# henrique/rsba

Measured on AMD Instinct MI355X. Metric: residual+Jacobian evals/sec, higher is better.
Workload: dtype f64; 1 GPU; C4: rolling-shutter scene, 1000 frames x 2 poses, 100000 points, 2041284 observations, HORIZONTAL shutter, calibrated; observations_total=2041284, observations_this_rank=2041284, jacobian_cols=15, partition=single GPU

## Files before the change

rsba_amd/csrc/chol_plan.cpp:

```cpp
#include "chol_plan.hpp"

#include <algorithm>

namespace rsba {

int32_t CholHostPlan::slot_of(int i, int k) const {
  if (i == k) return slot_base[k];
  auto it = std::lower_bound(col[k].begin(), col[k].end(), i);
  return (it != col[k].end() && *it == i) ? slot_base[k] + 1 + (int32_t)(it - col[k].begin()) : -1;
}

void chol_symbolic(int nt, const std::vector<std::vector<int32_t>>& adj, const TileOrder& order, CholHostPlan* hp) {
  hp->nt = nt;
  hp->perm = order.perm;
  const std::vector<int32_t>& perm = hp->perm;
  std::vector<int32_t>& iperm = hp->iperm;
  iperm.resize(nt);
  for (int k = 0; k < nt; ++k) iperm[perm[k]] = k;
  std::vector<std::vector<int32_t>>&col = hp->col, &row = hp->row;
  col.assign(nt, {}); row.assign(nt, {});
  {
    std::vector<std::vector<uint8_t>> mark(nt);
    for (int k = 0; k < nt; ++k) mark[k].assign(nt - k, 0);
    for (int t = 0; t < nt; ++t) for (int u : adj[t]) { const int i = std::max(iperm[t], iperm[u]), k = std::min(iperm[t], iperm[u]); mark[k][i - k] = 1; }
// ... 111 lines not shown
        s.sub_pub[fs] = (int32_t)(s.diag_info.size() / 4) - 1;
      } else s.diag_fuse.push_back(-1);
      sub_base[j] = (int32_t)(s.sub_info.size() / 4);
      s.back_info.push_back(slot_base[j]); s.back_info.push_back(perm[j]);
      for (auto it = col[j].rbegin(); it != col[j].rend(); ++it) { s.back_list.push_back(slot_of(*it, j)); s.back_list.push_back(perm[*it]); }
      s.back_ptr.push_back((int32_t)(s.back_list.size() / 2));
      for (int32_t i : col[j]) {
        s.sub_info.push_back(slot_of(i, j)); s.sub_info.push_back(slot_base[j]); s.sub_col.push_back(perm[j]); s.sub_pub.push_back(-1);
        if (sharded) { s.sub_info_sh.push_back(slot_of(i, j)); s.sub_info_sh.push_back(slot_base[j]); }
        sub_colnew.push_back(j);
        const int32_t sp0 = (int32_t)(s.sub_list.size() / 2);
        klev.clear(); pk.clear();
        for (int32_t k : rj) { const int32_t sik = slot_of(i, k); if (sik >= 0) { s.sub_list.push_back(sik); s.sub_list.push_back(slot_of(j, k)); klev.push_back(level[k]); if (topcol && cpart[k] >= 0) pk.push_back(cpart[k]); } }
        s.sub_ptr.push_back((int32_t)(s.sub_list.size() / 2));
        chunk_it(1, sp0, (int32_t)(s.sub_list.size() / 2), s.sub_info, s.sub_own, sp0, (int)pk.size(), pk, sharded ? &s.sub_info_sh : nullptr, slot_of(i, j));
      }
    }
    s.lev_diag_ptr.push_back((int32_t)(s.diag_info.size() / 4));
    s.lev_sub_ptr.push_back((int32_t)(s.sub_info.size() / 4));
    s.lev_upd_ptr.push_back((int32_t)(s.upd.size() / 4));
  }
  s.nparts = parts;
  auto push = [](std::vector<int32_t>& t, int kind, int item) { t.push_back(kind); t.push_back(item); };
  for (int l = 0; l < nlev; ++l) {
    for (int32_t u : upd_by_level[l]) push(s.tasks, kTaskUpdate, u);
    for (int d = s.lev_diag_ptr[l]; d < s.lev_diag_ptr[l + 1]; ++d) push(s.tasks, kTaskDiag, d);
    if (two_rhs) for (int d = s.lev_diag_ptr[l]; d < s.lev_diag_ptr[l + 1]; ++d) push(s.tasks, kTaskFwd2, d);
    for (int t = s.lev_sub_ptr[l]; t < s.lev_sub_ptr[l + 1]; ++t) push(s.tasks, kTaskSub, t);
  }
  if (two_rhs) push(s.tasks, kTaskEta, 0);
  for (int l = nlev - 1; l >= 0; --l)
    for (int d = s.lev_diag_ptr[l]; d < s.lev_diag_ptr[l + 1]; ++d) push(s.tasks, kTaskBack, d);
  s.diag_toprow.assign(diag_colnew.size(), -1);
  const int64_t T3 = (int64_t)kTile * kTile * kTile;
  s.cholesky_flops = T3 * ((int64_t)(s.diag_list.size() / 2) + 2 * (int64_t)(s.sub_list.size() / 2) + (int64_t)(s.sub_info.size() / 4)) +
                     2 * T3 / 3 * (int64_t)(s.diag_info.size() / 4) + 4 * (int64_t)kTile * kTile * ((int64_t)s.nslots + nt);
  s.row_mine.assign((size_t)nt, 1);
  if (!sharded) return;

  const int me = in.rank;
  auto mine_or_top = [&](int col_new, int kind, int item) { const int p = cpart[col_new]; if (p == me) push(s.tasks_a, kind, item); else if (p < 0) push(s.tasks_b, kind, item); };
  for (int l = 0; l < nlev; ++l) {
    for (int32_t u : upd_by_level[l]) { if (upd_owner[u] == me) push(s.tasks_a, kTaskUpdate, u); else if (upd_owner[u] < 0) push(s.tasks_b, kTaskUpdate, u); }
    for (int d = s.lev_diag_ptr[l]; d < s.lev_diag_ptr[l + 1]; ++d) mine_or_top(diag_colnew[d], kTaskDiag, d);
    if (two_rhs) for (int d = s.lev_diag_ptr[l]; d < s.lev_diag_ptr[l + 1]; ++d) mine_or_top(diag_colnew[d], kTaskFwd2, d);
    for (int t = s.lev_sub_ptr[l]; t < s.lev_sub_ptr[l + 1]; ++t) mine_or_top(sub_colnew[t], kTaskSub, t);
  }
  if (two_rhs) {
    for (int d = 0; d < (int)diag_colnew.size(); ++d) if (cpart[diag_colnew[d]] < 0) push(s.tasks_a, kTaskFwd2P, d);
    push(s.tasks_a, kTaskEta, 0);
    push(s.tasks_b, kTaskEta, 0);
  }
  for (int l = nlev - 1; l >= 0; --l)
    for (int d = s.lev_diag_ptr[l]; d < s.lev_diag_ptr[l + 1]; ++d) { const int p = cpart[diag_colnew[d]]; if (p == me || p < 0) push(s.tasks_b, kTaskBack, d); }
  {
    std::vector<int32_t> trow_of_col((size_t)nt, -1);
    int32_t cnt = 0;
    for (int j = 0; j < nt; ++j) if (cpart[j] < 0) trow_of_col[j] = cnt++;
    for (size_t d = 0; d < diag_colnew.size(); ++d) s.diag_toprow[d] = trow_of_col[diag_colnew[d]];
  }
  std::vector<uint8_t> has_pair((size_t)s.nslots, 0);
  for (size_t t = 0; t < in.pair_I->size(); ++t) { const int a = s.iperm[(*in.pair_I)[t]], b = s.iperm[(*in.pair_J)[t]]; has_pair[slot_of(std::max(a, b), std::min(a, b))] = 1; }
  s.asm_ptr.assign(1, 0);
  for (int j = 0; j < nt; ++j) if (cpart[j] < 0) {
    const int trow = (int)s.top_tiles.size();
    s.top_tiles.push_back(perm[j]);
    auto add = [&](int32_t slot, int rhs_row) {
      s.top_slots.push_back(slot); s.top_info.push_back(has_pair[slot]); s.top_info.push_back(rhs_row);
      const std::vector<int32_t>& a = asm_of_slot[slot];
      for (size_t q = 0; q + 1 < a.size(); q += 2) if (a[q] == me) s.asm_list.push_back(a[q + 1]);
// ... 16 lines not shown
```

rsba_amd/csrc/chol_plan.hpp:

```cpp
#pragma once
#include <cstdint>
#include <vector>

#include "tile_order.hpp"

namespace rsba {

enum : int { kTaskUpdate = 0, kTaskDiag = 1, kTaskSub = 2, kTaskBack = 3, kTaskFwd2 = 4, kTaskEta = 5, kTaskFwd2P = 6 };

struct CholPlanOptions {
  int chunk = 12, tail = 2;
  bool fuse_last = true;
};

struct CholTaskInput {
  const TileOrder* order = nullptr;
  bool sharded = false;
  int rank = 0;
  bool two_rhs = false;
  const std::vector<int32_t>*pair_I = nullptr, *pair_J = nullptr;
  CholPlanOptions opt;
};

struct CholHostPlan {
  int nt = 0, nslots = 0;
  std::vector<int32_t> perm, iperm;
  std::vector<std::vector<int32_t>> col, row;
  std::vector<int32_t> slot_base;
  std::vector<int32_t> slot_tiles;
  int32_t slot_of(int i, int k) const;

  bool sharded = false, two_rhs = false;
  int nlev = 0, nparts = 0;
  std::vector<int32_t> level, cpart;
  std::vector<int32_t> lev_diag_ptr, lev_sub_ptr, lev_upd_ptr;
  std::vector<int32_t> upd, upd_owner;
  std::vector<int32_t> diag_info, diag_ptr, diag_list, diag_own;
  std::vector<int32_t> diag_fuse;
  std::vector<int32_t> sub_info, sub_ptr, sub_list, sub_own;
  std::vector<int32_t> sub_col;
  std::vector<int32_t> sub_pub;
  std::vector<int32_t> back_info, back_ptr, back_list;
  std::vector<int32_t> tasks;
  std::vector<int32_t> fwd_full, diag_toprow;
  std::vector<int32_t> tasks_a, tasks_b, fwd_a, fwd_b;
  std::vector<int32_t> diag_info_sh, sub_info_sh;
  std::vector<int32_t> top_slots, top_info;
  std::vector<int32_t> asm_ptr, asm_list;
  std::vector<int32_t> top_tiles, top_fill;
  std::vector<uint8_t> row_mine, row_check, row_sep;
  int64_t cholesky_flops = 0;
  int local_levels = 0, separator_levels = 0;
};

void chol_symbolic(int nt, const std::vector<std::vector<int32_t>>& adj, const TileOrder& order, CholHostPlan* hp);
void chol_tasks(const CholTaskInput& in, CholHostPlan* hp);

}
```

rsba_amd/csrc/cholesky.hip:

```cpp
#include "solver_state.hpp"

namespace rsba {

namespace {

constexpr int T = kTile;
constexpr int TP = T + 1;

__device__ __forceinline__ double rsqrt_nr(double x) {
  double y = __builtin_amdgcn_rsq(x);
  y = y * (1.5 - 0.5 * x * y * y);
  y = y * (1.5 - 0.5 * x * y * y);
  return y;
}

__device__ __forceinline__ double* tile_ptr(const SolverDev& sv, int slot) { return sv.S + (size_t)slot * (T * T); }

__device__ __forceinline__ double readlane_f64(double v, int lane) {
  const int lo = __builtin_amdgcn_readlane(__double2loint(v), lane);
  const int hi = __builtin_amdgcn_readlane(__double2hiint(v), lane);
  return __hiloint2double(hi, lo);
}

__device__ __forceinline__ void lds_barrier() {
// ... 928 lines not shown
  switch (kind) {
    case kTaskUpdate: task_update<DAG>(sv, pl, item, smem, tid); break;
    case kTaskDiag: task_diag<DAG>(sv, pl, item, smem, tid); break;
    case kTaskSub: task_sub<DAG>(sv, pl, item, smem, tid); break;
    case kTaskFwd2: { const int tr = gl(pl.diag_toprow + item);
      task_forward<DAG>(sv, pl, item, gl(pl.fwd_range + 2 * item), gl(pl.fwd_range + 2 * item + 1), sv.border2, (pl.fwd2_minus && tr >= 0) ? pl.fwd2_minus + (size_t)tr * T : nullptr, sv.zv2, smem, tid); } break;
    case kTaskFwd2P: task_forward<DAG>(sv, pl, item, gl(pl.fwd_range + 2 * item), gl(pl.fwd_range + 2 * item + 1), sv.border2, nullptr, sv.zv2, smem, tid, pl.fwd2_partial + (size_t)gl(pl.diag_toprow + item) * T); break;
    case kTaskEta: task_eta<DAG>(sv, pl, smem, tid); break;
    default: task_back<DAG>(sv, pl, item, smem, tid); break;
  }
}

__global__ __launch_bounds__(256) void chol_level_kernel(const SolverDev sv, const CholPlan pl, int kind, int first) {
  extern __shared__ __attribute__((aligned(16))) double smem[];
  run_task<false>(sv, pl, kind, first + blockIdx.x, smem, threadIdx.x);
}

__global__ __launch_bounds__(256, 2) void chol_dag_kernel(const DagArgs* __restrict__ args) {
  extern __shared__ __attribute__((aligned(16))) double smem[];
  __shared__ int s_ticket;
  const int tid = threadIdx.x;
  const CholPlan& pl = args->pl;
  if (lm_stopped(args->sv.ctl)) return;
  for (;;) {
    lds_barrier();
    if (tid == 0) {
      const int tk = (int)__hip_atomic_fetch_add(pl.ticket, 1u, __ATOMIC_RELAXED, __HIP_MEMORY_SCOPE_AGENT);
      s_ticket = tk;
      s_trace_slot = (pl.trace && tk < pl.ntasks) ? pl.trace + 8 * (size_t)tk : nullptr;
      if (s_trace_slot) { s_trace_slot[0] = blockIdx.x; s_trace_slot[1] = s_trace_slot[2] = wall_clock64(); }
    }
    lds_barrier();
    const int t = s_ticket;
    if (t >= pl.ntasks) {
      if (tid == 0 && __hip_atomic_fetch_add(pl.ticket + 3, 1u, __ATOMIC_RELAXED, __HIP_MEMORY_SCOPE_AGENT) == gridDim.x - 1) {
        __hip_atomic_store(pl.ticket + 0, 0u, __ATOMIC_RELAXED, __HIP_MEMORY_SCOPE_AGENT);
        __hip_atomic_store(pl.ticket + 3, 0u, __ATOMIC_RELAXED, __HIP_MEMORY_SCOPE_AGENT);
      }
      return;
    }
    int task_tid = tid;
    asm volatile("" : "+v"(task_tid));
    run_task<true>(args->sv, pl, gl(pl.tasks + 2 * t), gl(pl.tasks + 2 * t + 1), smem, task_tid);
    if (tid == 0 && s_trace_slot) s_trace_slot[7] = wall_clock64();
  }
}

template <bool DAG>
__device__ __forceinline__ void task_forward(const SolverDev& sv, const CholPlan& pl, int d, int p0, int p1, const double* __restrict__ b2, const double* __restrict__ minus, double* z2,
                                             double* smem, int tid, double* partial_out) {
  constexpr int CG = 10;
  double* zb = smem;
  double* sp = smem + T;
// ... 228 lines not shown
```

rsba_amd/csrc/partition.hip:

```cpp
#include <algorithm>
#include <cstring>
#include <vector>

#include "handle.hpp"
#include "solver_state.hpp"
#include "tile_order.hpp"
#include "chol_plan.hpp"

using namespace rsba;

namespace {

int32_t partition(const rsba_problem_desc* d, int32_t world, int32_t* owner, int32_t* num_top_tiles, std::vector<int32_t>& part_of) {
  if (!d || !owner || world < 1) return rsba_set_error(RSBA_ERR_INVALID_ARGUMENT, "bad partition arguments");
  const int P = d->poses_per_frame;
  if (P != 1 && P != 2) return rsba_set_error(RSBA_ERR_INVALID_ARGUMENT, "poses_per_frame must be 1 or 2");
  const TileLayout lay(P, d->num_frames, d->calibrated != 0, d->num_intrinsics);
  const int FR = lay.FR, M = d->num_points, NIB = lay.NIB, NPF = lay.NPF, nt = lay.nt;
  const int64_t N = d->num_observations;
  if (num_top_tiles) *num_top_tiles = 0;
  if (world == 1 || N == 0) { std::fill(owner, owner + M, 0); part_of.assign(nt, 0); return RSBA_OK; }
  for (int64_t i = 0; i < N; ++i)
    if (d->obs_frame[i] < 0 || d->obs_frame[i] >= FR || d->obs_point[i] < 0 || d->obs_point[i] >= M) return rsba_set_error(RSBA_ERR_INVALID_ARGUMENT, "observation index out of range");
  auto intr_of = [&](int f) { return (NIB > 1 && d->frame_intrinsics) ? d->frame_intrinsics[f] : 0; };
// ... 69 lines not shown
}

extern "C" int32_t rsba_debug_chol_plan(int32_t nt, int32_t num_edges, const int32_t* edges, int32_t world, int32_t rank, int32_t two_rhs, int32_t chunk, int32_t tail,
                                        int32_t fuse_last, void (*emit)(void* ctx, const char* name, const int32_t* data, int64_t count), void* ctx) {
  if (nt < 1 || num_edges < 0 || (num_edges && !edges) || world < 1 || rank < 0 || rank >= world || tail < 1 || chunk < tail || !emit) return rsba_set_error(RSBA_ERR_INVALID_ARGUMENT, "bad plan arguments");
  std::vector<std::vector<int32_t>> adj(nt);
  std::vector<int32_t> pair_I, pair_J;
  for (int t = 0; t < nt; ++t) { pair_I.push_back(t); pair_J.push_back(t); }
  for (int e = 0; e < num_edges; ++e) {
    const int a = edges[2 * e], b = edges[2 * e + 1];
    if (a < 0 || a >= nt || b < 0 || b >= nt || a == b) return rsba_set_error(RSBA_ERR_INVALID_ARGUMENT, "bad edge");
    adj[a].push_back(b); adj[b].push_back(a);
  }
  for (int t = 0; t < nt; ++t) {
    std::sort(adj[t].begin(), adj[t].end()); adj[t].erase(std::unique(adj[t].begin(), adj[t].end()), adj[t].end());
    for (int32_t u : adj[t]) if (u < t) { pair_I.push_back(t); pair_J.push_back(u); }
  }
  const TileOrder ord = nested_dissection(nt, adj, plan_leaf_size(world, nt), world);
  CholHostPlan hp;
  chol_symbolic(nt, adj, ord, &hp);
  CholTaskInput in;
  in.order = &ord; in.sharded = world > 1 && ord.parts_ok; in.rank = rank; in.two_rhs = two_rhs != 0; in.pair_I = &pair_I; in.pair_J = &pair_J;
  in.opt.chunk = chunk; in.opt.tail = tail; in.opt.fuse_last = fuse_last != 0;
  chol_tasks(in, &hp);
  const std::vector<int32_t> meta{hp.sharded, hp.nlev, hp.nparts, hp.nslots};
  emit(ctx, "meta", meta.data(), (int64_t)meta.size());
  auto bytes = [&](const char* name, const std::vector<uint8_t>& v) { const std::vector<int32_t> w(v.begin(), v.end()); emit(ctx, name, w.data(), (int64_t)w.size()); };
#define RSBA_EMIT(x) emit(ctx, #x, hp.x.data(), (int64_t)hp.x.size())
  RSBA_EMIT(perm); RSBA_EMIT(slot_tiles); RSBA_EMIT(level); RSBA_EMIT(cpart); RSBA_EMIT(lev_diag_ptr); RSBA_EMIT(lev_sub_ptr); RSBA_EMIT(lev_upd_ptr);
  RSBA_EMIT(upd); RSBA_EMIT(upd_owner); RSBA_EMIT(diag_info); RSBA_EMIT(diag_ptr); RSBA_EMIT(diag_list); RSBA_EMIT(diag_own); RSBA_EMIT(diag_fuse);
  RSBA_EMIT(sub_info); RSBA_EMIT(sub_ptr); RSBA_EMIT(sub_list); RSBA_EMIT(sub_own); RSBA_EMIT(sub_col); RSBA_EMIT(sub_pub);
  RSBA_EMIT(back_info); RSBA_EMIT(back_ptr); RSBA_EMIT(back_list); RSBA_EMIT(tasks); RSBA_EMIT(fwd_full); RSBA_EMIT(diag_toprow);
  RSBA_EMIT(tasks_a); RSBA_EMIT(tasks_b); RSBA_EMIT(fwd_a); RSBA_EMIT(fwd_b); RSBA_EMIT(diag_info_sh); RSBA_EMIT(sub_info_sh);
  RSBA_EMIT(top_slots); RSBA_EMIT(top_info); RSBA_EMIT(asm_ptr); RSBA_EMIT(asm_list); RSBA_EMIT(top_tiles); RSBA_EMIT(top_fill);
#undef RSBA_EMIT
  bytes("row_mine", hp.row_mine); bytes("row_check", hp.row_check); bytes("row_sep", hp.row_sep);
  return RSBA_OK;
}
#endif
```

rsba_amd/csrc/solver.hip:

```cpp
#include <algorithm>
#include <chrono>
#include <cstdlib>
#include <cmath>
#include <cstdio>
#include <cstring>
#include <functional>
#include <limits>
#include <string>
#include <condition_variable>
#include <deque>
#include <memory>
#include <mutex>
#include <thread>
#include <unordered_map>
#include <vector>

#include "handle.hpp"
#include "devmem.hpp"
#include "solver_state.hpp"
#include "tile_order.hpp"
#include "chol_plan.hpp"
#include "plan_device.hpp"
#include "pcg.hpp"
#include "test_hooks.hpp"
// ... 32 lines not shown
  {&CholHostPlan::diag_toprow, &CholPlan::diag_toprow, kPlanAll},
};
constexpr size_t kNumPlanLists = sizeof kPlanLists / sizeof kPlanLists[0];

struct Solver {
  PhaseTimer timer;
  PhaseTimer xtimer;
  rsba_plan_stats stats{};
  SolverDev sv{};
  std::vector<void*> allocs;
  CholHostPlan hp;
  int32_t* d_plan_lists[kNumPlanLists] = {};
  DagArgs* d_dag_args = nullptr;
  int32_t* d_slot_tiles = nullptr;
  double* d_verify = nullptr;
  hipStream_t vstream = nullptr; hipEvent_t ev_solved = nullptr, ev_verified = nullptr; double* verify_b = nullptr; bool verify_pending = false;
  bool verify_dag = true;
  bool test_corrupt_once = false;
  int dag_fallbacks = 0;
  unsigned int* d_dag_sync = nullptr;
  long long* d_trace = nullptr;
  CholPlan plan{};
  int dag_workgroups = 0;
  bool dag_one_per_cu = true;
  bool use_levels = false;
  uint8_t* d_row_sep = nullptr;
  int32_t* d_obs_slot = nullptr;
  double *d_gpose = nullptr, *d_gpoint = nullptr;
  int64_t num_pairs = 0;
  double* cells[2] = {nullptr, nullptr}; size_t ncells = 0, cell_off[5] = {0, 0, 0, 0, 0};
  DagArgs* d_dag_args2[2] = {nullptr, nullptr};
  int cur_cells = 0;
  hipStream_t mstream = nullptr; hipEvent_t ev_armed[2] = {nullptr, nullptr}, ev_released = nullptr; bool arm_pending[2] = {false, false};
  hipEvent_t ev_fork = nullptr, ev_join = nullptr;
  int64_t schur_launches = 0;
  double* d_ctl = nullptr;
  rsba_iteration* d_trace_it = nullptr; int trace_it_cap = 0;
  static constexpr int kCtlRing = 4;
  bool clamp_with_factor = false; double clamp_lo_hi[2] = {0.0, 0.0};
  double* h_ctl = nullptr; double* h_ctl_dev = nullptr;
  bool gradmax_done = false;
  double ctl_seq = 0.0;
  bool sharded_off = false;
  CholPlan plan_a{}, plan_b{}; DagArgs* d_dag_args_a[2] = {nullptr, nullptr}; DagArgs* d_dag_args_b[2] = {nullptr, nullptr};
  int ntop_slots = 0, ntop_tiles = 0;
  int32_t *d_top_slots = nullptr, *d_top_info = nullptr, *d_asm_ptr = nullptr, *d_asm_list = nullptr, *d_top_tiles = nullptr;
  double* topx_buf = nullptr;
// ... 558 lines not shown
  if (sharded && !h->prior_frames.empty() && !h->prior_split) {
    auto part_of_frame = [&](int f) { return tord.part_of[f / FT]; };
    std::vector<int32_t> own((size_t)FR + 1, 0);
    int mine = 0;
    for (int32_t f : h->prior_frames) {
      int r = part_of_frame(f);
      if (r < 0) r = part_of_frame(f - 1);
      if (r < 0) r = 0;
      if (r == h->rank) { own[f] = 1; ++mine; }
    }
    int32_t* d_own = nullptr;
    if (int32_t rc_ = s_upload(s, &d_own, own)) return rc_;
    h->prior_of_all = h->dp.prior_of; h->prior_invalid_all = h->prior_invalid;
    h->dp.prior_of = d_own;
    if (h->prior_invalid > 0) h->prior_invalid = mine;
    h->prior_split = true;
  }
  CholTaskInput tin;
  tin.order = &tord; tin.sharded = sharded; tin.rank = h->rank; tin.pair_I = &tp_I; tin.pair_J = &tp_J;
  tin.two_rhs = h->prior_free && !h->prior_frames.empty();
  if (const char* e = std::getenv("RSBA_CHOL_FUSE")) tin.opt.fuse_last = e[0] != '0';
  if (const char* e = std::getenv("RSBA_CHOL_TAIL")) tin.opt.tail = std::max(1, std::atoi(e));
  if (const char* e = std::getenv("RSBA_CHOL_CHUNK")) tin.opt.chunk = std::max(tin.opt.tail, std::atoi(e));
  chol_tasks(tin, &hp);
  const bool two_rhs = hp.two_rhs;
  tick("tasks");
  std::vector<int32_t> chunk_tp, chunk_n; std::vector<int64_t> chunk_e0;
  std::vector<std::vector<int32_t>> pair_chunks(ntp);
  auto number_chunks = [&](int64_t kBlock) {
    chunk_tp.clear(); chunk_n.clear(); chunk_e0.clear();
    for (auto& pc : pair_chunks) pc.clear();
    if (dev_plan && kBlock < M) {
      const size_t nseg = dpo.seg_pair.size();
      std::vector<int32_t> order(nseg);
      for (size_t q = 0; q < nseg; ++q) order[q] = (int32_t)q;
      std::stable_sort(order.begin(), order.end(), [&](int32_t a, int32_t b) { return dpo.seg_block[a] != dpo.seg_block[b] ? dpo.seg_block[a] < dpo.seg_block[b] : dpo.seg_pair[a] < dpo.seg_pair[b]; });
      for (int32_t q : order) {
        const int tp_ = dpo.seg_pair[q];
        const int64_t q0 = dpo.seg_start[q], q1 = ((size_t)q + 1 < nseg && dpo.seg_pair[q + 1] == tp_) ? dpo.seg_start[q + 1] : tp_ptr[tp_ + 1];
        for (int64_t a = q0; a < q1; a += kSchurChunk) {
          pair_chunks[tp_].push_back((int32_t)chunk_tp.size());
          chunk_tp.push_back(tp_); chunk_e0.push_back(a); chunk_n.push_back((int32_t)std::min<int64_t>(kSchurChunk, q1 - a));
        }
      }
      return;
    }
// ... 322 lines not shown
    if ((rc = s_upload_const(s, &s->pp.tile_diag_slot, tds))) return rc;
  }
  HIP_TRY(hipMemset(sv.scalars, 0, 16 * sizeof(double)));
  HIP_TRY(hipMemset(sv.chol_fail, 0, sizeof(int)));
  CholPlan& pl = s->plan;
  pl.ntasks = (int)(hp.tasks.size() / 2); pl.ndiag = (int)(hp.diag_info.size() / 4);
  pl.ticket = s->d_dag_sync;
  pl.nslots = sv.nslots; pl.nparts = hp.nparts;
  if (sharded) {
    s->plan_a = pl; s->plan_a.ntasks = (int)(hp.tasks_a.size() / 2);
    s->plan_b = pl; s->plan_b.ntasks = (int)(hp.tasks_b.size() / 2);
    if (two_rhs) {
      double* tail = s->topx_buf + (size_t)s->ntop_slots * kTile * kTile + (size_t)s->ntop_tiles * kTile;
      s->plan_a.fwd2_partial = tail; s->plan_a.eta_tiles = s->d_row_check; s->plan_a.eta_partial = tail + (size_t)s->ntop_tiles * kTile;
      s->plan_b.fwd2_minus = tail; s->plan_b.eta_tiles = s->d_row_sep; s->plan_b.eta_extra = tail + (size_t)s->ntop_tiles * kTile;
    }
  }
  {
    CholPlan* const plans[3] = {&s->plan, &s->plan_a, &s->plan_b};
    for (size_t i = 0; i < kNumPlanLists; ++i) for (int b = 0; b < (sharded ? 3 : 1); ++b) if (kPlanLists[i].plans & (1u << b)) plans[b]->*kPlanLists[i].field = s->d_plan_lists[i];
  }
  int cus = 0;
  HIP_TRY(hipDeviceGetAttribute(&cus, hipDeviceAttributeMultiprocessorCount, h->device));
  s->dag_workgroups = std::max(1, std::min(pl.ntasks, std::max(cus, 1)));
  const int64_t my_tasks = sharded ? (int64_t)s->plan_a.ntasks + s->plan_b.ntasks : (int64_t)pl.ntasks;
  if (hp.nlev > 0 && my_tasks > (int64_t)hp.nlev * std::max(cus, 1)) { s->dag_workgroups = std::max(1, std::min(pl.ntasks, 2 * std::max(cus, 1))); s->dag_one_per_cu = false; }
  if (pl.ntasks <= 512) s->dag_workgroups = std::max(1, std::min(s->dag_workgroups, std::max(64, pl.ntasks / 4)));
  if (const char* e = std::getenv("RSBA_CHOL_WGS")) { s->dag_workgroups = std::max(1, std::min(std::min(pl.ntasks, 2 * std::max(cus, 1)), std::atoi(e))); s->dag_one_per_cu = s->dag_workgroups <= cus; }
  if (std::getenv("RSBA_CHOL_TRACE")) {
    if ((rc = s_alloc(s, &s->d_trace, 8 * (size_t)pl.ntasks))) return rc;
    HIP_TRY(hipMemset(s->d_trace, 0, 8 * (size_t)pl.ntasks * sizeof(long long)));
  }
  pl.trace = s->d_trace;
  tick("allocations");
  if (dbg_plan)
    std::fprintf(stderr, "[rsba plan] tiles %d, factor tiles %d, levels %d, tasks %d (partials %d); tile pairs %d, entries %lld, schur chunks %d\n", nt, sv.nslots,
                 hp.nlev, pl.ntasks, hp.nparts, sv.ntp, (long long)s->num_pairs, sv.nchunk);
  const char* lv = std::getenv("RSBA_CHOL_LEVELS");
  s->use_levels = lv && lv[0] == '1';
  {
    DagArgs host_args{sv, pl};
    if ((rc = s_upload(s, &s->d_slot_tiles, hp.slot_tiles))) return rc;
    if ((rc = s_alloc(s, &s->d_verify, 2 * (size_t)sv.npad))) return rc;
    if ((rc = s_alloc(s, &s->verify_b, (size_t)sv.npad))) return rc;
    HIP_TRY(dev_stream_acquire(&s->vstream));
    HIP_TRY(dev_event_acquire(&s->ev_solved, false));
    HIP_TRY(dev_event_acquire(&s->ev_verified, false));
    HIP_TRY(hipMemset(s->d_verify, 0, 2 * (size_t)sv.npad * sizeof(double)));
    { const char* v = std::getenv("RSBA_CHOL_VERIFY"); s->verify_dag = !(v && v[0] == '0'); }
    { const char* v = test_hook("RSBA_CHOL_TEST_CORRUPT"); s->test_corrupt_once = v && v[0] == '1'; }
    for (int b = 0; b < 2; ++b) {
// ... 180 lines not shown
int32_t await_verification(rsba_handle* h) {
  Solver* s = h->solver;
  if (s->verify_pending) { HIP_TRY(hipStreamWaitEvent(h->stream, s->ev_verified, 0)); s->verify_pending = false; }
  return RSBA_OK;
}
int32_t solve_reduced_system(rsba_handle* h, bool rhs_stays = false) {
  Solver* s = h->solver; SolverDev& sv = s->sv; hipStream_t st = h->stream;
  PhaseScope ps(h, RSBA_PHASE_CHOLESKY);
  if (int32_t rc = await_verification(h)) return rc;
  if (!s->use_levels) {
    const int used = s->cur_cells, now = used ^ 1;
    HIP_TRY(hipEventRecord(s->ev_released, st));
    HIP_TRY(hipStreamWaitEvent(s->mstream, s->ev_released, 0));
    HIP_TRY(hipMemsetAsync(s->cells[used], 0xFF, s->ncells * sizeof(double), s->mstream));
    HIP_TRY(hipEventRecord(s->ev_armed[used], s->mstream));
    s->arm_pending[used] = true;
    if (s->arm_pending[now]) { HIP_TRY(hipStreamWaitEvent(st, s->ev_armed[now], 0)); s->arm_pending[now] = false; }
    s->cur_cells = now;
    double* c = s->cells[now];
    sv.Lf = c + s->cell_off[0]; sv.chol_part = c + s->cell_off[1]; sv.Winv = c + s->cell_off[2]; sv.zv = c + s->cell_off[3]; sv.yv = sv.zv + sv.npad; sv.Xpub = c + s->cell_off[4];
    if (sv.zv2) { sv.zv2 = sv.zv + 2 * sv.npad; sv.ceta = sv.zv + 3 * sv.npad; }
    s->d_dag_args = s->d_dag_args2[now];
    if (s->hp.sharded && !s->sharded_off) {
      HIP_TRY(launch_chol_dag(sv, s->plan_a, s->d_dag_args_a[now], std::min(s->dag_workgroups, std::max(1, s->plan_a.ntasks)), s->dag_one_per_cu, st));
      const int64_t count = (int64_t)s->ntop_slots * kTile * kTile + (int64_t)s->ntop_tiles * kTile + (s->hp.two_rhs ? (int64_t)s->ntop_tiles * kTile + 8 : 0);
      ps.stop();
      {
        PhaseScope pe(h, RSBA_PHASE_EXCHANGE);
        HIP_TRY(launch_top_assemble(sv, s->d_top_slots, s->d_top_info, s->d_asm_ptr, s->d_asm_list, s->d_top_tiles, s->ntop_slots, s->topx_buf, st));
        if (int32_t rc = exchange(h, s->topx_buf, count, 0, RSBA_EXCHANGE_SYSTEM)) return rc;
        HIP_TRY(launch_top_unpack(sv, s->d_top_slots, s->d_top_info, s->d_top_tiles, s->ntop_slots, s->topx_buf, st));
      }
      ps.start();
      HIP_TRY(launch_chol_dag(sv, s->plan_b, s->d_dag_args_b[now], std::min(s->dag_workgroups, std::max(1, s->plan_b.ntasks)), s->dag_one_per_cu, st));
      ps.stop();
      {
        PhaseScope pe(h, RSBA_PHASE_EXCHANGE);
        HIP_TRY(launch_step_rows(sv.yv, s->d_row_mine, sv.npad, s->ybuf, st));
        if (int32_t rc = exchange(h, s->ybuf, sv.npad, 0, RSBA_EXCHANGE_STEP)) return rc;
        HIP_TRY(hipMemcpyAsync(sv.yv, s->ybuf, (size_t)sv.npad * sizeof(double), hipMemcpyDeviceToDevice, st));
      }
      ps.start();
    } else
    HIP_TRY(launch_chol_dag(sv, s->plan, s->d_dag_args, s->dag_workgroups, s->dag_one_per_cu, st));
    if (s->test_corrupt_once) { s->test_corrupt_once = false; HIP_TRY(hipMemsetAsync(sv.yv + (sv.n / 2 / 6) * 6 + 1, 0, sizeof(double), st)); }
    if (s->verify_dag) {
      const double* b_rhs = sv.rhs;
      if (s->hp.two_rhs) { HIP_TRY(launch_border_combine(s->verify_b, sv.rhs, s->border, 0.0, sv.npad, st, s->ratio4 + kRtC)); b_rhs = s->verify_b; }
      else if (!rhs_stays) { HIP_TRY(hipMemcpyAsync(s->verify_b, sv.rhs, (size_t)sv.npad * sizeof(double), hipMemcpyDeviceToDevice, st)); b_rhs = s->verify_b; }
      HIP_TRY(hipEventRecord(s->ev_solved, st));
      HIP_TRY(hipStreamWaitEvent(s->vstream, s->ev_solved, 0));
      HIP_TRY(launch_chol_verify(sv, s->d_slot_tiles, b_rhs, s->d_verify, s->d_verify + sv.npad, 1e-7, sv.scalars + kDagSuspect, s->vstream,
                                 s->hp.sharded && !s->sharded_off ? s->d_row_check : nullptr));
      HIP_TRY(hipEventRecord(s->ev_verified, s->vstream));
      s->verify_pending = true;
    }
  } else {
    for (int l = 0; l < s->hp.nlev; ++l) {
      const int d0 = s->hp.lev_diag_ptr[l], d1 = s->hp.lev_diag_ptr[l + 1], t0 = s->hp.lev_sub_ptr[l], t1 = s->hp.lev_sub_ptr[l + 1];
      const int u0 = s->hp.lev_upd_ptr[l], u1 = s->hp.lev_upd_ptr[l + 1];
      HIP_TRY(launch_chol_level(sv, s->plan, kTaskUpdate, u0, u1 - u0, st));
      HIP_TRY(launch_chol_level(sv, s->plan, kTaskDiag, d0, d1 - d0, st));
      if (s->hp.two_rhs) HIP_TRY(launch_chol_level(sv, s->plan, kTaskFwd2, d0, d1 - d0, st));
      HIP_TRY(launch_chol_level(sv, s->plan, kTaskSub, t0, t1 - t0, st));
    }
    if (s->hp.two_rhs) HIP_TRY(launch_chol_level(sv, s->plan, kTaskEta, 0, 1, st));
    for (int l = s->hp.nlev - 1; l >= 0; --l) {
// ... 407 lines not shown
      HIP_TRY(launch_own_points(dp, sv, s->merge_buf, st));
      int32_t rc2 = exchange(h, s->merge_buf, 4 * (int64_t)dp.M, 0, RSBA_EXCHANGE_POINTS);
      if (rc2) return rc2;
      HIP_TRY(launch_merge_points(dp, s->merge_buf, st));
    }
    HIP_TRY(hipMemcpyAsync(h->desc.poses, dp.poses, npose * sizeof(double), hipMemcpyDeviceToHost, st));
    HIP_TRY(hipMemcpyAsync(h->desc.points, dp.points, npt * sizeof(double), hipMemcpyDeviceToHost, st));
    if (!dp.calibrated) HIP_TRY(hipMemcpyAsync(h->desc.intrinsics, dp.intr, (size_t)dp.NI * 9 * sizeof(double), hipMemcpyDeviceToHost, st));
    if (dp.pp_count > 0 && h->pp_host) HIP_TRY(hipMemcpyAsync(h->pp_host, dp.pp_value, 6 * (size_t)dp.pp_count * sizeof(double), hipMemcpyDeviceToHost, st));
    HIP_TRY(hipStreamSynchronize(st));
    if (s->timer.on) { s->timer.resolve(); s->timer.on = false; }
    if (s->xtimer.on) { s->xtimer.resolve(); s->xtimer.on = false; }
    h->prior_ratio_result = dp.prior_ratio;
    sum->total_time_s = now_s() - t_start;
    if (const char* path = h->solver->d_trace ? std::getenv("RSBA_CHOL_TRACE") : nullptr) {
      Solver* sl = h->solver;
      std::vector<long long> tr(8 * (size_t)sl->plan.ntasks);
      HIP_TRY(hipMemcpy(tr.data(), sl->d_trace, tr.size() * sizeof(long long), hipMemcpyDeviceToHost));
      if (FILE* f = std::fopen(path, "wb")) {
        const int32_t n = sl->plan.ntasks;
        std::fwrite(&n, sizeof(n), 1, f);
        std::fwrite(sl->hp.tasks.data(), sizeof(int32_t), sl->hp.tasks.size(), f);
        std::fwrite(tr.data(), sizeof(long long), tr.size(), f);
        std::fclose(f);
      }
    }
    return RSBA_OK;
  };

  double t0 = now_s();
  if ((rc = reset_scales(h))) return rc;
  if ((rc = linearize(h, false, true))) return rc;
  if ((rc = gradient_max(h))) return rc;
  if ((rc = read_back())) return rc;
  sum->residual_jacobian_time_s += now_s() - t0;
  if (nfail) { sum->termination_type = RSBA_FAILURE; (void)finish(RSBA_FAILURE); return rsba_set_error(RSBA_ERR_EVALUATION_FAILED, "initial residual and Jacobian evaluation failed"); }
  double cost = cost2[0]; const double fixed = cost2[1];
  auto with_ratio_gradient = [&](double g) { return free_ratio ? std::max(g, std::fabs(ratio - std::max(ratio_lb, ratio - ratio_hg[1]))) : g; };
  double gmax = with_ratio_gradient(host_sc[kGradMax]);
  sum->fixed_cost = fixed; sum->initial_cost = cost + fixed; sum->final_cost = cost + fixed;
  double radius = opt->initial_trust_region_radius, decrease_factor = 2.0; bool reuse_diagonal = false;
  rsba_iteration it; std::memset(&it, 0, sizeof it);
  it.cost = cost + fixed; it.gradient_max_norm = gmax; it.trust_region_radius = radius;
  if (gmax <= opt->gradient_tolerance) { push(it); return finish(RSBA_CONVERGENCE); }
  if (opt->jacobi_scaling) {
    HIP_TRY(launch_jacobi_scale(dp, sv, st));
// ... 258 lines not shown
```

rsba_amd/csrc/solver_state.hpp:

```cpp
#pragma once
#include <hip/hip_runtime.h>
#include <cstdint>

#include "../../include/rsba_amd.h"
#include "device_state.hpp"
#include "chol_plan.hpp"

namespace rsba {

constexpr int kSchurChunk = 512;
constexpr int kMaxRankSlots = 64;
constexpr int kGroupFull = 3 * kTile;
constexpr int kGroupFactored = 80;

struct SolverDev {
  int F, Fx, NPF;
  int NIB;
  const int32_t* intr_frame_ptr;
  const int32_t* intr_frame_list;
  int64_t nvgroups;
  const int32_t* vgroup_point;
  const int32_t* vgroup_intr;
  const int64_t* point_vgroup;
  int CD;
// ... 87 lines not shown
  kRtDiagTerm = 4, kRtGs = 5, kRtScale = 6,
  kRtEta = 7, kRtC = 8,
  kRtRatio = 9, kRtRatioNew = 10, kRtDiag = 11, kRtLb = 12,
  kRtRatioEval = 13,
  kRtSize = 16
};

enum ScalarSlot : int {
  kModelCostChange = 0, kStepSq = 1, kXSq = 2, kGradMax = 3, kCost = 4, kFixedCost = 5, kEvalFailed = 6, kSolveFailed = 7,
  kDagSuspect = 11,
};

hipError_t allow_dynamic_lds_impl(const void* kernel, size_t bytes);
template <class K>
inline hipError_t allow_dynamic_lds(K kernel, size_t bytes) { return allow_dynamic_lds_impl(reinterpret_cast<const void*>(kernel), bytes); }

struct CholPlan {
  const int32_t *upd, *diag_info, *diag_ptr, *diag_list, *sub_info, *sub_ptr, *sub_list, *sub_col, *diag_own, *sub_own, *back_info, *back_ptr, *back_list;
  const int32_t* diag_fuse;
  const int32_t* sub_pub;
  int ndiag;
  const int32_t* tasks;
  int ntasks;
  unsigned int* ticket;
  long long* trace;
  int nslots, nparts;
  const int32_t* fwd_range;
  const int32_t* diag_toprow;
  const double* fwd2_minus;
  double* fwd2_partial;
  const uint8_t* eta_tiles;
  const double* eta_extra;
  double* eta_partial;
};

struct PosePriorDev {
  double *v0, *g0, *cross;
  double* diag;
  const int32_t* tile_diag_slot;
};
hipError_t launch_pose_prior_blocks(const DeviceProblem& dp, const SolverDev& sv, const PosePriorDev& pp, hipStream_t st);
hipError_t launch_pose_prior_scale(const DeviceProblem& dp, const PosePriorDev& pp, hipStream_t st);
hipError_t launch_pose_prior_clamp(const DeviceProblem& dp, const PosePriorDev& pp, double lo, double hi, hipStream_t st);
hipError_t launch_pose_prior_gradmax(const DeviceProblem& dp, const SolverDev& sv, const PosePriorDev& pp, hipStream_t st, double* out = nullptr);
hipError_t launch_pose_prior_take(const DeviceProblem& dp, const SolverDev& sv, hipStream_t st);
hipError_t launch_pose_prior_reduce(const DeviceProblem& dp, const SolverDev& sv, const PosePriorDev& pp, double radius, hipStream_t st);
// ... 61 lines not shown
```

Measured before the change: 18.83 billion obs evals/s.

## Split DAG Cholesky workgroups into hosts and guests that stop at narrow levels

Computes the per-level task width of the Cholesky DAG and a 'narrow_from' task index, then launches the DAG kernel with a host count capped at the CU count plus optional guest workgroups. Guests pull tickets only until the queue reaches the narrow tail, so extra workgroups do not contend on the ticket atomic or spin on narrow levels. Grid sizing per plan (full, sharded A and B) replaces the single workgroup count, and the trace now records hardware placement. By default narrow_from is INT_MAX for wide plans and 0 otherwise, which mostly reproduces the old sizing. The metric here is residual and Jacobian throughput, which this solver-side change barely touches.

```diff
diff --git a/rsba_amd/csrc/chol_plan.cpp b/rsba_amd/csrc/chol_plan.cpp
--- a/rsba_amd/csrc/chol_plan.cpp
+++ b/rsba_amd/csrc/chol_plan.cpp
@@ -157,12 +157,23 @@
   }
   s.nparts = parts;
   auto push = [](std::vector<int32_t>& t, int kind, int item) { t.push_back(kind); t.push_back(item); };
-  for (int l = 0; l < nlev; ++l) {
+  auto narrow = [&](const std::vector<int32_t>& lev_ptr, const std::vector<int32_t>& width) {
+    int32_t from = 0;
+    for (int l = 0; l < nlev; ++l) if (width[l] >= in.opt.width) from = lev_ptr[l + 1];
+    return from;
+  };
+  std::vector<int32_t> width(nlev, 0);
+  for (int l = 0; l < nlev; ++l) width[l] = (s.lev_diag_ptr[l + 1] - s.lev_diag_ptr[l]) + (s.lev_sub_ptr[l + 1] - s.lev_sub_ptr[l]) + (s.lev_upd_ptr[l + 1] - s.lev_upd_ptr[l]);
+  for (int l = 0; l < nlev; ++l) {
+    s.lev_task_ptr.push_back((int32_t)(s.tasks.size() / 2));
     for (int32_t u : upd_by_level[l]) push(s.tasks, kTaskUpdate, u);
     for (int d = s.lev_diag_ptr[l]; d < s.lev_diag_ptr[l + 1]; ++d) push(s.tasks, kTaskDiag, d);
     if (two_rhs) for (int d = s.lev_diag_ptr[l]; d < s.lev_diag_ptr[l + 1]; ++d) push(s.tasks, kTaskFwd2, d);
     for (int t = s.lev_sub_ptr[l]; t < s.lev_sub_ptr[l + 1]; ++t) push(s.tasks, kTaskSub, t);
   }
+  s.lev_task_ptr.push_back((int32_t)(s.tasks.size() / 2));
+  s.narrow_from.assign(3, 0);
+  s.narrow_from[0] = narrow(s.lev_task_ptr, width);
   if (two_rhs) push(s.tasks, kTaskEta, 0);
   for (int l = nlev - 1; l >= 0; --l)
     for (int d = s.lev_diag_ptr[l]; d < s.lev_diag_ptr[l + 1]; ++d) push(s.tasks, kTaskBack, d);
@@ -175,12 +186,21 @@
 
   const int me = in.rank;
   auto mine_or_top = [&](int col_new, int kind, int item) { const int p = cpart[col_new]; if (p == me) push(s.tasks_a, kind, item); else if (p < 0) push(s.tasks_b, kind, item); };
-  for (int l = 0; l < nlev; ++l) {
+  std::vector<int32_t> width_a(nlev, 0), width_b(nlev, 0);
+  for (int l = 0; l < nlev; ++l) {
+    for (int d = s.lev_diag_ptr[l]; d < s.lev_diag_ptr[l + 1]; ++d) { const int p = cpart[diag_colnew[d]]; width_a[l] += p == me; width_b[l] += p < 0; }
+    for (int t = s.lev_sub_ptr[l]; t < s.lev_sub_ptr[l + 1]; ++t) { const int p = cpart[sub_colnew[t]]; width_a[l] += p == me; width_b[l] += p < 0; }
+    for (int u = s.lev_upd_ptr[l]; u < s.lev_upd_ptr[l + 1]; ++u) { width_a[l] += upd_owner[u] == me; width_b[l] += upd_owner[u] < 0; }
+  }
+  for (int l = 0; l < nlev; ++l) {
+    s.lev_task_ptr_a.push_back((int32_t)(s.tasks_a.size() / 2)); s.lev_task_ptr_b.push_back((int32_t)(s.tasks_b.size() / 2));
     for (int32_t u : upd_by_level[l]) { if (upd_owner[u] == me) push(s.tasks_a, kTaskUpdate, u); else if (upd_owner[u] < 0) push(s.tasks_b, kTaskUpdate, u); }
     for (int d = s.lev_diag_ptr[l]; d < s.lev_diag_ptr[l + 1]; ++d) mine_or_top(diag_colnew[d], kTaskDiag, d);
     if (two_rhs) for (int d = s.lev_diag_ptr[l]; d < s.lev_diag_ptr[l + 1]; ++d) mine_or_top(diag_colnew[d], kTaskFwd2, d);
     for (int t = s.lev_sub_ptr[l]; t < s.lev_sub_ptr[l + 1]; ++t) mine_or_top(sub_colnew[t], kTaskSub, t);
   }
+  s.lev_task_ptr_a.push_back((int32_t)(s.tasks_a.size() / 2)); s.lev_task_ptr_b.push_back((int32_t)(s.tasks_b.size() / 2));
+  s.narrow_from[1] = narrow(s.lev_task_ptr_a, width_a); s.narrow_from[2] = narrow(s.lev_task_ptr_b, width_b);
   if (two_rhs) {
     for (int d = 0; d < (int)diag_colnew.size(); ++d) if (cpart[diag_colnew[d]] < 0) push(s.tasks_a, kTaskFwd2P, d);
     push(s.tasks_a, kTaskEta, 0);
diff --git a/rsba_amd/csrc/chol_plan.hpp b/rsba_amd/csrc/chol_plan.hpp
--- a/rsba_amd/csrc/chol_plan.hpp
+++ b/rsba_amd/csrc/chol_plan.hpp
@@ -11,6 +11,7 @@
 struct CholPlanOptions {
   int chunk = 12, tail = 2;
   bool fuse_last = true;
+  int width = 128;
 };
 
 struct CholTaskInput {
@@ -44,6 +45,7 @@
   std::vector<int32_t> tasks;
   std::vector<int32_t> fwd_full, diag_toprow;
   std::vector<int32_t> tasks_a, tasks_b, fwd_a, fwd_b;
+  std::vector<int32_t> lev_task_ptr, lev_task_ptr_a, lev_task_ptr_b, narrow_from;
   std::vector<int32_t> diag_info_sh, sub_info_sh;
   std::vector<int32_t> top_slots, top_info;
   std::vector<int32_t> asm_ptr, asm_list;
diff --git a/rsba_amd/csrc/cholesky.hip b/rsba_amd/csrc/cholesky.hip
--- a/rsba_amd/csrc/cholesky.hip
+++ b/rsba_amd/csrc/cholesky.hip
@@ -974,13 +974,21 @@
   const int tid = threadIdx.x;
   const CholPlan& pl = args->pl;
   if (lm_stopped(args->sv.ctl)) return;
+  const bool guest = (int)blockIdx.x >= pl.hosts;
   for (;;) {
     lds_barrier();
     if (tid == 0) {
-      const int tk = (int)__hip_atomic_fetch_add(pl.ticket, 1u, __ATOMIC_RELAXED, __HIP_MEMORY_SCOPE_AGENT);
+      int tk = pl.ntasks;
+      if (!guest || (int)__hip_atomic_load(pl.ticket, __ATOMIC_RELAXED, __HIP_MEMORY_SCOPE_AGENT) < pl.narrow_from)
+        tk = (int)__hip_atomic_fetch_add(pl.ticket, 1u, __ATOMIC_RELAXED, __HIP_MEMORY_SCOPE_AGENT);
       s_ticket = tk;
       s_trace_slot = (pl.trace && tk < pl.ntasks) ? pl.trace + 8 * (size_t)tk : nullptr;
-      if (s_trace_slot) { s_trace_slot[0] = blockIdx.x; s_trace_slot[1] = s_trace_slot[2] = wall_clock64(); }
+      if (s_trace_slot) {
+        const unsigned hw = __builtin_amdgcn_s_getreg((4 << 0) | (8 << 6) | (7 << 11)), xcc = __builtin_amdgcn_s_getreg((20 << 0) | (0 << 6) | (3 << 11));
+        const unsigned where = (xcc << 8) | hw;
+        s_trace_slot[0] = (long long)blockIdx.x | (long long)where << 32;
+        s_trace_slot[1] = s_trace_slot[2] = wall_clock64();
+      }
     }
     lds_barrier();
     const int t = s_ticket;
diff --git a/rsba_amd/csrc/partition.hip b/rsba_amd/csrc/partition.hip
--- a/rsba_amd/csrc/partition.hip
+++ b/rsba_amd/csrc/partition.hip
@@ -115,6 +115,7 @@
   CholTaskInput in;
   in.order = &ord; in.sharded = world > 1 && ord.parts_ok; in.rank = rank; in.two_rhs = two_rhs != 0; in.pair_I = &pair_I; in.pair_J = &pair_J;
   in.opt.chunk = chunk; in.opt.tail = tail; in.opt.fuse_last = fuse_last != 0;
+  if (const char* e = std::getenv("RSBA_CHOL_WIDTH")) in.opt.width = std::max(1, std::atoi(e));
   chol_tasks(in, &hp);
   const std::vector<int32_t> meta{hp.sharded, hp.nlev, hp.nparts, hp.nslots};
   emit(ctx, "meta", meta.data(), (int64_t)meta.size());
@@ -125,6 +126,7 @@
   RSBA_EMIT(sub_info); RSBA_EMIT(sub_ptr); RSBA_EMIT(sub_list); RSBA_EMIT(sub_own); RSBA_EMIT(sub_col); RSBA_EMIT(sub_pub);
   RSBA_EMIT(back_info); RSBA_EMIT(back_ptr); RSBA_EMIT(back_list); RSBA_EMIT(tasks); RSBA_EMIT(fwd_full); RSBA_EMIT(diag_toprow);
   RSBA_EMIT(tasks_a); RSBA_EMIT(tasks_b); RSBA_EMIT(fwd_a); RSBA_EMIT(fwd_b); RSBA_EMIT(diag_info_sh); RSBA_EMIT(sub_info_sh);
+  RSBA_EMIT(lev_task_ptr); RSBA_EMIT(lev_task_ptr_a); RSBA_EMIT(lev_task_ptr_b); RSBA_EMIT(narrow_from);
   RSBA_EMIT(top_slots); RSBA_EMIT(top_info); RSBA_EMIT(asm_ptr); RSBA_EMIT(asm_list); RSBA_EMIT(top_tiles); RSBA_EMIT(top_fill);
 #undef RSBA_EMIT
   bytes("row_mine", hp.row_mine); bytes("row_check", hp.row_check); bytes("row_sep", hp.row_sep);
diff --git a/rsba_amd/csrc/solver.hip b/rsba_amd/csrc/solver.hip
--- a/rsba_amd/csrc/solver.hip
+++ b/rsba_amd/csrc/solver.hip
@@ -1,4 +1,5 @@
 #include <algorithm>
+#include <climits>
 #include <chrono>
 #include <cstdlib>
 #include <cmath>
@@ -78,7 +79,7 @@
   long long* d_trace = nullptr;
   CholPlan plan{};
   int dag_workgroups = 0;
-  bool dag_one_per_cu = true;
+  int dag_grid[3] = {0, 0, 0}; bool dag_one_per_cu[3] = {true, true, true};
   bool use_levels = false;
   uint8_t* d_row_sep = nullptr;
   int32_t* d_obs_slot = nullptr;
@@ -683,6 +684,8 @@
   if (const char* e = std::getenv("RSBA_CHOL_FUSE")) tin.opt.fuse_last = e[0] != '0';
   if (const char* e = std::getenv("RSBA_CHOL_TAIL")) tin.opt.tail = std::max(1, std::atoi(e));
   if (const char* e = std::getenv("RSBA_CHOL_CHUNK")) tin.opt.chunk = std::max(tin.opt.tail, std::atoi(e));
+  { int ncu = 0; HIP_TRY(hipDeviceGetAttribute(&ncu, hipDeviceAttributeMultiprocessorCount, h->device)); tin.opt.width = std::max(1, ncu / 2); }
+  if (const char* e = std::getenv("RSBA_CHOL_WIDTH")) tin.opt.width = std::max(1, std::atoi(e));
   chol_tasks(tin, &hp);
   const bool two_rhs = hp.two_rhs;
   tick("tasks");
@@ -1051,11 +1054,30 @@
   }
   int cus = 0;
   HIP_TRY(hipDeviceGetAttribute(&cus, hipDeviceAttributeMultiprocessorCount, h->device));
-  s->dag_workgroups = std::max(1, std::min(pl.ntasks, std::max(cus, 1)));
+  const int ncu = std::max(cus, 1);
   const int64_t my_tasks = sharded ? (int64_t)s->plan_a.ntasks + s->plan_b.ntasks : (int64_t)pl.ntasks;
-  if (hp.nlev > 0 && my_tasks > (int64_t)hp.nlev * std::max(cus, 1)) { s->dag_workgroups = std::max(1, std::min(pl.ntasks, 2 * std::max(cus, 1))); s->dag_one_per_cu = false; }
+  const bool wide_plan = hp.nlev > 0 && my_tasks > (int64_t)hp.nlev * ncu;
+  {
+    const int cap = pl.ntasks <= 512 ? std::max(64, pl.ntasks / 4) : 2 * ncu;
+    const char *e_wgs = std::getenv("RSBA_CHOL_WGS"), *e_hosts = std::getenv("RSBA_CHOL_HOSTS"), *e_narrow = std::getenv("RSBA_CHOL_NARROW"), *e_guests = std::getenv("RSBA_CHOL_GUESTS");
+    const bool by_plan = e_guests && e_guests[0] == '1';
+    CholPlan* const plans[3] = {&pl, &s->plan_a, &s->plan_b};
+    for (int b = 0; b < (sharded ? 3 : 1); ++b) {
+      CholPlan& p = *plans[b];
+      p.hosts = std::max(1, std::min(std::min(p.ntasks, ncu), cap));
+      p.narrow_from = by_plan ? hp.narrow_from[b] : wide_plan ? INT_MAX : 0;
+      if (e_narrow) { const int v = std::atoi(e_narrow); p.narrow_from = v < 0 ? INT_MAX : v; }
+      int grid = p.narrow_from > 0 ? std::max(p.hosts, std::min(std::min(by_plan ? INT_MAX : std::max(p.ntasks, 1), 2 * ncu), cap)) : p.hosts;
+      if (e_wgs) grid = std::max(1, std::min(2 * ncu, std::atoi(e_wgs)));
+      if (e_hosts) p.hosts = std::max(1, std::atoi(e_hosts));
+      p.hosts = std::min(p.hosts, grid);
+      s->dag_grid[b] = grid; s->dag_one_per_cu[b] = grid <= p.hosts && grid <= ncu;
+    }
+  }
+  s->dag_workgroups = std::max(1, std::min(pl.ntasks, ncu));
+  if (wide_plan) s->dag_workgroups = std::max(1, std::min(pl.ntasks, 2 * ncu));
   if (pl.ntasks <= 512) s->dag_workgroups = std::max(1, std::min(s->dag_workgroups, std::max(64, pl.ntasks / 4)));
-  if (const char* e = std::getenv("RSBA_CHOL_WGS")) { s->dag_workgroups = std::max(1, std::min(std::min(pl.ntasks, 2 * std::max(cus, 1)), std::atoi(e))); s->dag_one_per_cu = s->dag_workgroups <= cus; }
+  if (const char* e = std::getenv("RSBA_CHOL_WGS")) s->dag_workgroups = std::max(1, std::min(std::min(pl.ntasks, 2 * ncu), std::atoi(e)));
   if (std::getenv("RSBA_CHOL_TRACE")) {
     if ((rc = s_alloc(s, &s->d_trace, 8 * (size_t)pl.ntasks))) return rc;
     HIP_TRY(hipMemset(s->d_trace, 0, 8 * (size_t)pl.ntasks * sizeof(long long)));
@@ -1282,7 +1304,7 @@
     if (sv.zv2) { sv.zv2 = sv.zv + 2 * sv.npad; sv.ceta = sv.zv + 3 * sv.npad; }
     s->d_dag_args = s->d_dag_args2[now];
     if (s->hp.sharded && !s->sharded_off) {
-      HIP_TRY(launch_chol_dag(sv, s->plan_a, s->d_dag_args_a[now], std::min(s->dag_workgroups, std::max(1, s->plan_a.ntasks)), s->dag_one_per_cu, st));
+      HIP_TRY(launch_chol_dag(sv, s->plan_a, s->d_dag_args_a[now], s->dag_grid[1], s->dag_one_per_cu[1], st));
       const int64_t count = (int64_t)s->ntop_slots * kTile * kTile + (int64_t)s->ntop_tiles * kTile + (s->hp.two_rhs ? (int64_t)s->ntop_tiles * kTile + 8 : 0);
       ps.stop();
       {
@@ -1292,7 +1314,7 @@
         HIP_TRY(launch_top_unpack(sv, s->d_top_slots, s->d_top_info, s->d_top_tiles, s->ntop_slots, s->topx_buf, st));
       }
       ps.start();
-      HIP_TRY(launch_chol_dag(sv, s->plan_b, s->d_dag_args_b[now], std::min(s->dag_workgroups, std::max(1, s->plan_b.ntasks)), s->dag_one_per_cu, st));
+      HIP_TRY(launch_chol_dag(sv, s->plan_b, s->d_dag_args_b[now], s->dag_grid[2], s->dag_one_per_cu[2], st));
       ps.stop();
       {
         PhaseScope pe(h, RSBA_PHASE_EXCHANGE);
@@ -1302,7 +1324,7 @@
       }
       ps.start();
     } else
-    HIP_TRY(launch_chol_dag(sv, s->plan, s->d_dag_args, s->dag_workgroups, s->dag_one_per_cu, st));
+    HIP_TRY(launch_chol_dag(sv, s->plan, s->d_dag_args, s->dag_grid[0], s->dag_one_per_cu[0], st));
     if (s->test_corrupt_once) { s->test_corrupt_once = false; HIP_TRY(hipMemsetAsync(sv.yv + (sv.n / 2 / 6) * 6 + 1, 0, sizeof(double), st)); }
     if (s->verify_dag) {
       const double* b_rhs = sv.rhs;
@@ -1756,6 +1778,8 @@
         std::fwrite(&n, sizeof(n), 1, f);
         std::fwrite(sl->hp.tasks.data(), sizeof(int32_t), sl->hp.tasks.size(), f);
         std::fwrite(tr.data(), sizeof(long long), tr.size(), f);
+        const int32_t sizing[3] = {sl->dag_grid[0], sl->plan.hosts, sl->plan.narrow_from};
+        std::fwrite(sizing, sizeof(int32_t), 3, f);
         std::fclose(f);
       }
     }
diff --git a/rsba_amd/csrc/solver_state.hpp b/rsba_amd/csrc/solver_state.hpp
--- a/rsba_amd/csrc/solver_state.hpp
+++ b/rsba_amd/csrc/solver_state.hpp
@@ -133,6 +133,7 @@
   int ndiag;
   const int32_t* tasks;
   int ntasks;
+  int hosts, narrow_from;
   unsigned int* ticket;
   long long* trace;
   int nslots, nparts;
```

Measured after the change: 18.61 billion obs evals/s. -1.2%, worse.
